# 0x002A/MuCHSALSA

Measured on AMD Instinct MI355X. Metric: overlap-pairs/s, higher is better.
Workload: dtype int32+f64; 1 GPU; 100k synthetic Nanopore x10 kb, 500k unitig anchors, 10x coverage (BASELINE.json configs[2]); rows=5059558, reads=100000, anchors=499992, edges=981460, edgematches_rank0=25532466, orders_rank0=1029308, parallelism=one job on one GPU, edges_proven_clean_rank0=5372

## Files before the change

### muchsalsa_amd/csrc/msgpu_api.hip

```cpp
#include <hip/hip_runtime.h>

#include <chrono>
#include <cmath>
#include <cstdarg>
#include <cstdio>
#include <cstdlib>
#include <cstring>
#include <condition_variable>
#include <deque>
#include <mutex>
#include <new>
#include <thread>
#include <vector>
#include <algorithm>
#include <sys/mman.h>
#include <unistd.h>

#include "asm_internal.h"
#include "host_pool.h"
#include "msgpu.h"
#include "msgpu_internal.h"
#include "msgpu_stage.h"

using namespace msgpu;
// ... 189 lines not shown
}

struct msgpu_ctx : msgpu::StageCtx {
  hipStream_t  own_stream = nullptr;
  msgpu_params p;
  State        state      = ST_CREATED;
  uint32_t     shard = 0, nshards = 1;
  uint32_t     win_lo = 0, win_hi = 0xffffffffu;
  uint64_t     base_edges = 0, base_ems = 0, base_orders = 0, base_ids = 0;
  ScalarBlock  sc;
  bool         stage_events = true;
  bool         chain_zeroed = false;
  bool         no_prologue = false;
  bool         prologue_ok = false;
  bool         scalars_clean = false;
  bool         bin_clean = false;
  size_t       bin_zero_words = 0;
  uint32_t     prologue_shard = 0, prologue_nshards = 1;
  uint64_t     prologue_own = 0;
  bool         full_scan_ok = false;
  uint64_t     index_total = 0, own_accum = 0;
  bool         nlists_clean = false;
  bool         cand_zeroed = false;
  uint64_t     prologue_bound = 0;
  uint32_t     prologue_lists[4] = {0, 0, 0, 0};
  EventHold    ev_order;
  uint32_t     decl_V = 0, decl_A = 0;
  bool                                  has_deadline = false;
  std::chrono::steady_clock::time_point deadline{};

  uint64_t n_rows = 0, n_alive = 0;
  uint32_t V = 0, A = 0;
  const msgpu_row *d_rows = nullptr;

  uint64_t n_edges = 0, n_ems = 0, n_orders = 0, n_ids = 0, n_visit = 0, total_bound = 0;
  uint32_t n_list[4] = {0, 0, 0, 0};

  DevBuf rows_in, rows_pk, cnt_read, read_off, cursor, bkt_key, bkt_dead, by_read, read_cnt, alive_rank,
      anchor_cnt, anchor_off, anchor_first, anchor_off_gen, bkt2_idx, bkt2_line, by_anchor, read_len, read_first,
      scan_tmp, vis16, spos2, visits, bin_cursor, bin_start;
  DevBuf bound, cand_off, cand_j, cand_q, scr_v2, scr_start, n_cand, n_edge, lists, edges, edge_cand;
  DevBuf big_key, big_t, big_r2s, big_pfx, pair_tab, chain_chunks, big_off, cand_sums, bucket_visits;
  EventHold ev_side[2], ev_side2;
  uint64_t    n_big_edges = 0, n_big_ems = 0;
  bool   fast_path = true;
  bool   chain_band = true;
  bool   sub_wave  = true;
  bool   use_fork  = true;
  bool   use_prologue = true;
  bool   chain_serial = false;
  uint32_t n_cls[4] = {0, 0, 0, 0};
  uint64_t n_edges_fast = 0;
  uint64_t chain_E = 0;
  DevBuf ems, order_scr, ids_scr, edge_norders, edge_nids, orders, ids, big_list, cls_list, big_elems,
      big_paths;
  DevBuf g_deg, g_off, g_adj, g_cand, g_sane, g_out;
  DevBuf sel_idx, sel_cnt, sel_off, sel_ems;

  DevBuf    alt_edges, alt_ems, alt_orders, alt_ids;
  EventHold ev_done[2], ev_copied[2];
  HostBuf   h_edges, h_ems, h_orders, h_ids, h_read_len, h_read_first, h_sel_off, h_sel_ems, h_wire[2];
  EventHold ev_part[2][3];
  std::mutex              gate_m;
  std::condition_variable gate_cv;
  uint64_t                chain_launches = 0;
  DevBuf win_cuts;
  DevBuf wire_dev[2];
  bool   wire_copy = true;

  EventHold ev[10];
  static constexpr int CK_RING = 256;
  EventHold  ck_ev[CK_RING][2];
  uint32_t   ck_head = 0, ck_count = 0;
  bool       have_index_t = false, have_cand_t = false, have_chain_t = false, index_fast = false;
  bool   have_stage_t = false;
  uint32_t index_path = 0;
  bool     index_binned = false;
  bool     use_bin = true;
  StreamHold side_stream, side_stream2, copy_stream;
  int        open() {
    own_stream = stream;
    if (int rc = sc.create()) return rc;
    const char *nf = getenv("MSGPU_NO_FASTPATH");
    fast_path      = !(nf && nf[0] == '1');
    const char *nb = getenv("MSGPU_NO_BAND");
    chain_band     = fast_path && !(nb && nb[0] == '1');
    const char *ns = getenv("MSGPU_NO_SUBWAVE");
    sub_wave       = !(ns && ns[0] == '1');
    const char *nw = getenv("MSGPU_NO_WIRE_COPY");
    wire_copy      = !(nw && nw[0] == '1');
    const char *nbin = getenv("MSGPU_NO_BIN");
    use_bin          = !(nbin && nbin[0] == '1');
    use_prologue = !getenv("MSGPU_NO_PROLOGUE");
    use_fork     = !getenv("MSGPU_NO_FORK");
    chain_serial = getenv("MSGPU_CHAIN_SERIAL") != nullptr;
    int prio_least = 0, prio_greatest = 0;
    if (hipDeviceGetStreamPriorityRange(&prio_least, &prio_greatest) != hipSuccess) prio_least = prio_greatest = 0;
    bool ok = side_stream.create(hipStreamNonBlocking, prio_greatest) == hipSuccess &&
              side_stream2.create(hipStreamNonBlocking, prio_greatest) == hipSuccess && copy_stream.create() == hipSuccess;
    for (auto &e : ev) ok = ok && e.create() == hipSuccess;
    EventHold *const untimed[] = {&ev_order, &ev_side[0], &ev_side[1], &ev_side2, &ev_done[0], &ev_done[1], &ev_copied[0], &ev_copied[1],
                                  &ev_part[0][0], &ev_part[0][1], &ev_part[0][2], &ev_part[1][0], &ev_part[1][1], &ev_part[1][2]};
    for (EventHold *e : untimed) ok = ok && e->create(hipEventDisableTiming) == hipSuccess;
    return ok ? MSGPU_OK : MSGPU_E_HIP;
  }
};

// ... 661 lines not shown
    k.pub            = publish ? c->sc.arm() : HostPublish{nullptr, 0};
    k.nlists         = scalar<unsigned long long>(c, SC_NLISTS);
    launch_emit_edges(st, k, publish);
  };
  uint64_t cap_edges = 0, cap_big = 0;
  capacities(&cap_edges, &cap_big);
  emit(cap_edges, cap_big, true);
  c->nlists_clean = true;
  STAGE_HIP(c, hipGetLastError());
  if (int rc = close_readback(c)) return rc;
  const uint64_t *tot = host_scalar<uint64_t>(c, SC_TOTAL_A), *big = host_scalar<uint64_t>(c, SC_BIGSTATS);
  c->n_big_edges = big[0];
  c->n_big_ems   = big[1];
  for (int k = 0; k < 4; ++k) c->n_cls[k] = host_scalar<uint32_t>(c, SC_CLS)[k];
  c->n_ems   = tot[0];
  c->n_edges = tot[1];
  c->n_visit = c->total_bound;
  if (c->n_edges >= 0xfffffff0ull) return fail(c, MSGPU_E_ARG, "edge table too large (%llu)", (unsigned long long)c->n_edges);
  if (c->n_edges > cap_edges || c->n_big_edges >= cap_big) {
    STAGE_HIP(c, c->edges.ensure((c->n_edges ? c->n_edges : 1) * sizeof(msgpu_edge)));
    STAGE_HIP(c, c->edge_cand.ensure((c->n_edges ? c->n_edges : 1) * 8));
    STAGE_HIP(c, c->cls_list.ensure((c->n_edges + 1) * 4));
    STAGE_HIP(c, c->big_list.ensure((c->n_big_edges + 1) * 4));
    STAGE_HIP(c, c->big_off.ensure((c->n_big_edges + 1) * 8));
    STAGE_HIP(c, c->chain_chunks.ensure(chunk_words(c->edges.room() / sizeof(msgpu_edge)) * 8));
    capacities(&cap_edges, &cap_big);
    emit(cap_edges, cap_big, false);
  }
  c->chain_zeroed = true;
  STAGE_HIP(c, hipGetLastError());
  if (c->stage_events) STAGE_HIP(c, hipEventRecord(c->ev[3], st));
  c->have_cand_t = c->stage_events;
  c->n_orders    = 0;
  c->n_ids       = 0;
  c->state       = ST_EDGES;
  return MSGPU_OK;
}

int msgpu_chaining_and_overlaps(msgpu_ctx *c) {
  if (!c) return MSGPU_E_ARG;
  if (c->state < ST_EDGES || c->state == ST_RESULT)
    return fail(c, MSGPU_E_STATE, "msgpu_chaining_and_overlaps before msgpu_calculate_edges");
  STAGE_HIP(c, hipSetDevice(c->device));
  hipStream_t    st = c->stream;
  const uint64_t E = c->n_edges, M = c->n_ems;
  for (int k = 0; k < 2; ++k)
    if (!c->ck_ev[c->ck_head][k]) STAGE_HIP(c, c->ck_ev[c->ck_head][k].create());
  const hipEvent_t ck_begin = c->ck_ev[c->ck_head][0], ck_end = c->ck_ev[c->ck_head][1];
  if (c->stage_events) STAGE_HIP(c, hipEventRecord(c->ev[4], st));

  STAGE_HIP(c, c->ems.ensure((M ? M : 1) * sizeof(msgpu_edgematch)));
  STAGE_HIP(c, c->order_scr.ensure((M ? M : 1) * sizeof(msgpu_order)));
  STAGE_HIP(c, c->ids_scr.ensure((M ? M : 1) * 4));
  STAGE_HIP(c, c->edge_norders.ensure((E + 4) * 4));
  STAGE_HIP(c, c->edge_nids.ensure((E + 4) * 4));
  STAGE_HIP(c, c->chain_chunks.ensure(chunk_words(E) * 8));

  ChainArgs a;
  a.edges        = c->edges.as<msgpu_edge>();
  a.edge_cand    = c->edge_cand.as<uint64_t>();
  a.n_edges      = E;
  a.cand_j       = c->cand_j.as<uint32_t>();
  a.cand_q       = c->cand_q.as<uint32_t>();
  a.read_off     = c->read_off.as<uint32_t>();
  a.read_cnt     = c->read_cnt.as<uint32_t>();
  a.read_len     = c->read_len.as<int32_t>();
  a.by_read      = c->by_read.as<IRow>();
  a.ems          = c->ems.as<msgpu_edgematch>();
  a.order_scr    = c->order_scr.as<msgpu_order>();
  a.ids_scr      = c->ids_scr.as<uint32_t>();
  a.edge_norders = c->edge_norders.as<uint32_t>();
  a.edge_nids    = c->edge_nids.as<uint32_t>();
  a.err          = scalar<uint32_t>(c, SC_ERR);
  if (!c->pair_tab.p) {
    STAGE_HIP(c, c->pair_tab.ensure(PAIR_TAB_WORDS * sizeof(uint32_t)));
    launch_fill_pair_tab(st, c->pair_tab.as<uint32_t>());
  }
  a.pair_tab     = c->pair_tab.as<uint32_t>();
  a.pair_tab64   = c->pair_tab.as<uint32_t>() + 4 * PAIR_TAB_STRIDE;
  a.pair_tab_sub = c->pair_tab.as<uint32_t>() + 4 * PAIR_TAB_STRIDE + 2 * PAIR_TAB_STRIDE;
  if (!c->chain_zeroed)
    STAGE_HIP(c, hipMemsetAsync(c->chain_chunks.p, 0, chunk_words(E) * 8, st));
  c->chain_zeroed = false;
  a.chunk_sums   = c->chain_chunks.as<unsigned long long>();
  a.fast_path    = (c->fast_path ? CHAIN_FAST_SHORTCUT : 0) | (c->chain_band ? CHAIN_FAST_BAND : 0);
  c->chain_E     = E;
  a.fast_margin  = static_cast<long long>(std::min<uint64_t>(c->p.wiggle_room, uint64_t(1) << 40)) - 3;
  a.wiggle       = static_cast<double>(c->p.wiggle_room);
  a.ratio_pct    = c->p.ratio_pct;
  a.alt_frac     = c->p.alt_frac;
  a.out_edge_base = static_cast<uint32_t>(c->base_edges);

  const uint32_t n_big = static_cast<uint32_t>(c->n_big_edges);
  if (n_big) {
    STAGE_HIP(c, c->big_elems.ensure((c->n_big_ems ? c->n_big_ems : 1) * big_elem_bytes()));
    STAGE_HIP(c, c->big_paths.ensure((c->n_big_ems ? c->n_big_ems : 1) * 2 * big_path_bytes()));
  }
  if (n_big) STAGE_HIP(c, hipEventRecord(c->ev_side[0], st));
  auto launch_big = [&]() -> int {
    if (!n_big) return MSGPU_OK;
    STAGE_HIP(c, hipStreamWaitEvent(c->side_stream, c->ev_side[0], 0));
    launch_chain_big(c->side_stream, a, c->big_list.as<uint32_t>(), c->big_off.as<uint64_t>(), n_big,
                     c->big_elems.p, c->big_paths.p);
    STAGE_HIP(c, hipEventRecord(c->ev_side[1], c->side_stream));
    return MSGPU_OK;
  };
  {
    std::lock_guard<std::mutex> g(c->gate_m);
    ++c->chain_launches;
  }
  c->gate_cv.notify_all();
  if (int rc = launch_big()) return rc;
  STAGE_HIP(c, hipEventRecord(ck_begin, st));
  if (c->sub_wave && E) {
    const uint32_t *list = c->cls_list.as<uint32_t>();
    const uint32_t *l64 = list, *l32 = l64 + c->n_cls[2], *l16 = l32 + c->n_cls[1], *l8 = l16 + c->n_cls[0];
    const bool serial = c->chain_serial;
    const bool any_sub = c->n_cls[0] || c->n_cls[1] || c->n_cls[3];
    const bool beside  = !serial && any_sub && c->n_cls[2];
    if (beside) STAGE_HIP(c, hipStreamWaitEvent(c->side_stream2, ck_begin, 0));
    launch_chain(st, a, l64, c->n_cls[2]);
    if (serial) {
      launch_chain_sub(st, a, 32, l32, c->n_cls[1]);
      launch_chain_sub(st, a, 16, l16, c->n_cls[0]);
      launch_chain_sub(st, a, 8, l8, c->n_cls[3]);
    } else if (any_sub) {
      launch_chain_sub_all(beside ? c->side_stream2 : st, a, l32, c->n_cls[1], l16, c->n_cls[0], l8, c->n_cls[3]);
    }
    if (beside) {
      STAGE_HIP(c, hipEventRecord(c->ev_side2, c->side_stream2));
      STAGE_HIP(c, hipStreamWaitEvent(st, c->ev_side2, 0));
    }
  } else {
    launch_chain(st, a, nullptr, 0);
  }
  STAGE_HIP(c, hipEventRecord(ck_end, st));
  c->ck_head = (c->ck_head + 1) % msgpu_ctx::CK_RING;
  if (c->ck_count < msgpu_ctx::CK_RING) ++c->ck_count;
  STAGE_HIP(c, hipGetLastError());
  if (n_big) STAGE_HIP(c, hipStreamWaitEvent(st, c->ev_side[1], 0));

  if (c->stage_events) STAGE_HIP(c, hipEventRecord(c->ev[7], st));
  auto compact = [&](bool publish) {
    CompactArgs k;
    k.edges        = c->edges.as<msgpu_edge>();
    k.n_edges      = E;
    k.edge_norders = c->edge_norders.as<uint32_t>();
    k.edge_nids    = c->edge_nids.as<uint32_t>();
    k.chunk_sums   = c->chain_chunks.as<unsigned long long>();
    k.n_chunks     = static_cast<uint32_t>((E + COMPACT_CHUNK - 1) / COMPACT_CHUNK);
    k.scalars      = c->sc.d;
    k.pub          = publish ? c->sc.arm() : HostPublish{nullptr, 0};
    k.order_scr    = c->order_scr.as<msgpu_order>();
    k.ids_scr      = c->ids_scr.as<uint32_t>();
    k.orders       = c->orders.as<msgpu_order>();
    k.ids          = c->ids.as<uint32_t>();
    k.out_em_base    = c->base_ems;
    k.out_order_base = c->base_orders;
    k.out_ids_base   = c->base_ids;
    k.out_edge_base  = static_cast<uint32_t>(c->base_edges);
    k.cap_orders     = c->orders.room() / sizeof(msgpu_order);
    k.cap_ids        = c->ids.room() / 4;
    launch_compact(st, k);
  };
  const uint64_t cap_orders = c->orders.room() / sizeof(msgpu_order), cap_ids = c->ids.room() / 4;
  compact(true);
  STAGE_HIP(c, hipGetLastError());
  if (int rc = close_readback(c)) return rc;
  c->n_edges_fast     = *host_scalar<uint64_t>(c, SC_TOTAL_C);
  const uint64_t *tot = host_scalar<uint64_t>(c, SC_TOTAL_A);
  c->n_orders = tot[0];
  c->n_ids    = tot[1];
  if (c->n_orders > cap_orders || c->n_ids > cap_ids) {
    STAGE_HIP(c, c->orders.ensure((c->n_orders ? c->n_orders : 1) * sizeof(msgpu_order)));
    STAGE_HIP(c, c->ids.ensure((c->n_ids ? c->n_ids : 1) * 4));
    compact(false);
  }
  STAGE_HIP(c, hipGetLastError());
  if (c->stage_events) STAGE_HIP(c, hipEventRecord(c->ev[8], st));
  c->have_chain_t = true;
  c->have_stage_t = c->stage_events;
  c->state        = ST_CHAINED;
  return MSGPU_OK;
}

int msgpu_set_stage_events(msgpu_ctx *c, int on) {
  if (!c) return MSGPU_E_ARG;
  c->stage_events = on != 0;
  return MSGPU_OK;
}

int msgpu_get_counts(msgpu_ctx *c, msgpu_counts *out) {
  if (!c || !out) return MSGPU_E_ARG;
  memset(out, 0, sizeof(*out));
  out->n_rows_in       = c->n_rows;
  out->n_rows_alive    = c->n_alive;
  out->n_reads         = c->V;
  out->n_anchors       = c->A;
  out->n_edges         = c->state >= ST_EDGES ? c->n_edges : 0;
  out->n_ems           = c->state >= ST_EDGES ? c->n_ems : 0;
  out->n_orders        = c->state >= ST_CHAINED ? c->n_orders : 0;
// ... 757 lines not shown
```

### muchsalsa_amd/csrc/msgpu_internal.h

```cpp
#ifndef MSGPU_INTERNAL_H
#define MSGPU_INTERNAL_H

#include <hip/hip_runtime.h>
#include <stdint.h>

#include "msgpu.h"

namespace msgpu {

struct IRow {
  int32_t  n_lo, n_hi, i_lo, i_hi;
  uint32_t score, line, other, pf;
};
static_assert(sizeof(IRow) == 32, "IRow must be 32 bytes");
struct SRow {
  int32_t  i_lo, i_hi;
  uint32_t read, pf;
};
static_assert(sizeof(SRow) == 16, "SRow must be 16 bytes");
constexpr uint32_t PF_POS_MASK = 0x3fffffffu;
constexpr uint32_t PF_DIR      = 1u << 30;
constexpr uint32_t PF_PRIM     = 1u << 31;

enum { SC_MAXIDS = 0 , SC_ERR = 1, SC_TOTAL_A = 2, SC_TOTAL_B = 3, SC_TOTAL_C = 4, SC_NLISTS = 5 ,
// ... 17 lines not shown
  const uint32_t *read_off, *read_cnt, *anchor_off;
  const IRow     *by_read;
  const SRow     *by_anchor;
  const uint4    *vis;
  const uint64_t *cand_off;
  uint32_t       *cand_j;
  uint32_t       *cand_q;
  uint32_t       *edge_scr_v2;
  uint32_t       *edge_scr_start;
  uint32_t       *n_cand, *n_edge;
  unsigned long long *big_stats;
  uint32_t        th_overlap;
};
constexpr uint32_t CAND_CHUNK = 256;
struct CandZero {
  uint32_t *n_cand, *n_edge;
  uint32_t *scalar_words;
  uint32_t  n_scalar_words;
};
struct EmitArgs {
  const uint32_t *n_edge, *n_cand;
  const uint64_t *cand_off;
  const uint32_t *edge_scr_v2, *edge_scr_start;
  uint32_t        V;
  const uint32_t *hist;
  const unsigned long long *chunk_sums;
  uint32_t        n_chunks;
  msgpu_edge     *edges;
  uint64_t       *edge_cand;
  uint32_t       *list;
  uint32_t       *big_list;
  uint64_t       *big_off;
  unsigned long long *big_cursor;
  const unsigned long long *big_stats;
  uint64_t        cap_edges, cap_big;
  unsigned long long *chain_chunk_sums;
  uint32_t        n_chain_chunk_words;
  uint64_t       *scalars;
  HostPublish     pub;
  unsigned long long *nlists;
};

struct ChainArgs {
  msgpu_edge      *edges;
  const uint64_t  *edge_cand;
  uint64_t         n_edges;
  const uint32_t  *cand_j, *cand_q;
  const uint32_t  *read_off, *read_cnt;
  const int32_t   *read_len;
  const IRow      *by_read;
  msgpu_edgematch *ems;
  msgpu_order     *order_scr;
  uint32_t        *ids_scr;
  uint32_t        *edge_norders, *edge_nids;
  uint32_t        *err;
  const uint32_t  *pair_tab;
  const uint32_t  *pair_tab64;
  const uint32_t  *pair_tab_sub;
  unsigned long long *chunk_sums;
  int              fast_path;
  long long        fast_margin;
  double           wiggle, ratio_pct, alt_frac;
  uint32_t         out_edge_base;
};

constexpr uint32_t COMPACT_CHUNK = 1024;
struct CompactArgs {
  msgpu_edge        *edges;
  uint64_t           n_edges;
  const uint32_t    *edge_norders, *edge_nids;
  const unsigned long long *chunk_sums;
  uint32_t           n_chunks;
  uint64_t          *scalars;
  HostPublish        pub;
  const msgpu_order *order_scr;
  const uint32_t    *ids_scr;
  msgpu_order       *orders;
  uint32_t          *ids;
  uint64_t           out_em_base, out_order_base, out_ids_base;
  uint32_t           out_edge_base;
  uint64_t           cap_orders, cap_ids;
};

constexpr uint32_t MAX_WORLD = 64;
struct MergeBase {
  uint64_t edges, orders, ids;
  uint32_t read_id, anchor_id;
};
struct MergeArgs {
  const uint8_t *gathered;
  uint64_t       slab_bytes, off_edges, off_orders, off_ids;
  uint32_t       world;
  MergeBase      base[MAX_WORLD + 1];
  msgpu_edge    *edges;
  msgpu_order   *orders;
  uint32_t      *ids;
};

struct PackWireArgs {
  const msgpu_edge  *edges;
  const msgpu_order *orders;
  const uint32_t    *ids;
  uint64_t           n_edges, n_orders, n_ids;
  uint8_t           *w_edges, *w_orders;
  uint32_t          *w_ids;
  uint64_t           base_ems = 0, base_orders = 0, base_ids = 0;
  uint32_t           base_edges = 0;
};
inline uint64_t wire_edges_bytes(uint64_t n) { return 17 * n + 8; }
inline uint64_t wire_orders_bytes(uint64_t n) { return 33 * n + 4; }
inline uint64_t wire_ids_bytes(uint64_t n, uint32_t id_bytes) { return id_bytes == 3 ? (3 * n + 3) / 4 * 4 : 4 * n; }
struct WindowCutArgs {
  uint32_t n;
  float    frac[255];
};
void launch_window_cuts(hipStream_t st, const uint64_t *cum, uint32_t V, const WindowCutArgs &a, uint64_t *out);
void launch_pack_wire(hipStream_t st, const PackWireArgs &a);
void unpack_wire_host(const uint8_t *w_edges, const uint8_t *w_orders, const uint32_t *w_ids, uint32_t id_bytes, uint64_t n_edges,
                      uint64_t n_orders, uint64_t n_ids, uint64_t base_edges, uint64_t base_ems, uint64_t base_orders,
                      uint64_t base_ids, msgpu_edge *edges, msgpu_order *orders, uint32_t *ids, unsigned threads, unsigned tables = 7);
void launch_merge_wire(hipStream_t st, const MergeArgs &a, bool ids3);

template <class T> void exclusive_scan(hipStream_t st, const uint32_t *in, uint64_t n, T *out, T *block_sums, T *d_total);
// ... 148 lines not shown
```

### muchsalsa_amd/csrc/msgpu_kernels.hip

```cpp
#include <hip/hip_runtime.h>
#include <stdint.h>
#include <stdlib.h>

#include <type_traits>
#include <utility>

#include "msgpu.h"
#include "msgpu_internal.h"
#include "msgpu_device.h"

namespace msgpu {


constexpr int SCAN_ITEMS = 8;
uint32_t      scan_blocks(uint64_t n);

template <class T> __global__ __launch_bounds__(256) void k_scan_reduce(const uint32_t *in, uint64_t n, T *block_sums) {
  __shared__ T s[4];
  uint64_t     base = static_cast<uint64_t>(blockIdx.x) * 256 * SCAN_ITEMS;
  T            sum  = 0;
  for (int i = 0; i < SCAN_ITEMS; ++i) {
    uint64_t idx = base + static_cast<uint64_t>(i) * 256 + threadIdx.x;
    if (idx < n) sum += in[idx];
  }
// ... 1246 lines not shown
    const uint32_t e = sub;
    st_r[round] = en_r[round] = v2_r[round] = 0;
    if (e < ne_r4[round]) {
      st_r[round] = a.edge_scr_start[co_r[round] + e];
      en_r[round] = (e + 1 < ne_r4[round]) ? a.edge_scr_start[co_r[round] + e + 1] : nc_r4[round];
      v2_r[round] = a.edge_scr_v2[co_r[round] + e];
    }
  }
#pragma unroll
  for (int round = 0; round < ROUNDS; ++round) {
    const uint32_t lr = round * 64 + (threadIdx.x >> 4), r = chunk * CAND_CHUNK + lr;
    const uint32_t ne = ne_r4[round];
    if (ne == 0) continue;
    const uint32_t nc = nc_r4[round];
    const uint64_t eb = base_e + s_eb[lr], mb = base_m + s_mb[lr], co = co_r[round];
    for (uint32_t e = sub; e < ne; e += 16) {
      const bool     first = e == static_cast<uint32_t>(sub);
      const uint32_t st = first ? st_r[round] : a.edge_scr_start[co + e];
      const uint32_t en = first ? en_r[round] : ((e + 1 < ne) ? a.edge_scr_start[co + e + 1] : nc);
      msgpu_edge     ed;
      ed.v1        = r;
      ed.v2        = first ? v2_r[round] : a.edge_scr_v2[co + e];
      ed.em_off    = mb + st;
      ed.order_off = 0;
      ed.em_cnt    = en - st;
      ed.order_cnt = 0;
      ed.shadow    = 0;
      ed.pad       = 0;
      a.edges[eb + e]     = ed;
      a.edge_cand[eb + e] = co + st;
      if (ed.em_cnt > 64) {
        const unsigned long long i = atomicAdd(&a.big_cursor[0], 1ull);
        a.big_list[i] = static_cast<uint32_t>(eb + e);
        a.big_off[i]  = atomicAdd(&a.big_cursor[1], static_cast<unsigned long long>(ed.em_cnt));
      } else if (ed.em_cnt) {
        a.list[atomicAdd(&s_pos[ed.em_cnt - 1], 1u)] = static_cast<uint32_t>(eb + e);
      }
    }
  }
}
void launch_emit_edges(hipStream_t st, const EmitArgs &a, bool reduce) {
  if (reduce && a.n_chunks)
    hipLaunchKernelGGL(k_cand_reduce, dim3(a.n_chunks), dim3(1024), 0, st, a.n_edge, a.n_cand, a.cand_off, a.edge_scr_start, a.V,
                       const_cast<unsigned long long *>(a.chunk_sums), const_cast<uint32_t *>(a.hist));
  hipLaunchKernelGGL(k_emit_edges, dim3(a.n_chunks ? a.n_chunks : 1), dim3(1024), 0, st, a);
}


__device__ __forceinline__ void chunk_add(unsigned long long *chunk_sums, uint64_t e, bool clean, uint32_t n_orders, uint32_t n_ids, bool banded = false) {
  static_assert(COMPACT_CHUNK < (1u << 16), "two 16-bit edge counts in the low half of a chunk sum");
  unsigned long long *c = chunk_sums + 2 * (e / COMPACT_CHUNK);
  __hip_atomic_fetch_add(c, (clean ? 1ull : 0ull) | (banded ? 1ull << 16 : 0ull) | (static_cast<unsigned long long>(n_orders) << 32), __ATOMIC_RELAXED, __HIP_MEMORY_SCOPE_AGENT);
  __hip_atomic_fetch_add(c + 1, static_cast<unsigned long long>(n_ids), __ATOMIC_RELAXED, __HIP_MEMORY_SCOPE_AGENT);
}
__device__ __forceinline__ void band_fallback_add(unsigned long long *chunk_sums, uint64_t n_edges) {
  __hip_atomic_fetch_add(chunk_sums + 2 * (n_edges / COMPACT_CHUNK + 1), 1ull, __ATOMIC_RELAXED, __HIP_MEMORY_SCOPE_AGENT);
}

struct PathRec {
  uint64_t mask;
  uint64_t score;
  uint32_t primary;
  uint32_t pad;
};

struct __attribute__((aligned(16))) ChainElem {
  double clo1, chi1;
  double clo2, chi2;
  int    rlo1, rhi1, rlo2, rhi2;
};

struct NanoMasks {
  unsigned long long pos, neg, ovl, abort_;
};
template <bool WF, int SORTED >
__device__ __forceinline__ NanoMasks nano_check(double k_clo, double k_chi, double l_clo, double l_chi, int k_rlo,
                                                int k_rhi, int l_rlo, int l_rhi, double &d) {
  typedef unsigned long long M;
  const bool lt_lo_b = k_clo < l_clo;
  const M    lt_lo = __ballot(lt_lo_b), lt_hi = __ballot(k_chi < l_chi);
  const M    gt_lo = __ballot(k_clo > l_clo), gt_hi = __ballot(k_chi > l_chi);
  NanoMasks  f;
  const double x = k_chi - l_clo;
  const double y = l_chi - k_clo;
  double       t = lt_lo_b ? x : y;
  if (WF) {
    f.ovl = __ballot(t >= 0.0);
    d     = fabs(t) + 1;
  } else {
    f.ovl = __ballot(k_clo <= l_chi) & __ballot(l_clo <= k_chi);
    t     = __builtin_amdgcn_inverse_ballot_w64(f.ovl) ? t : -t;
    d = t + 1;
  }
  if (WF) {
    f.pos = lt_lo & lt_hi;
    f.neg = gt_lo & gt_hi;
  } else {
    f.pos = lt_lo & (lt_hi | ~f.ovl);
    f.neg = (f.ovl & gt_lo & gt_hi) | ~(f.ovl | lt_lo);
  }
  if (SORTED == 1) {
    const M rovl = __ballot(l_rlo <= k_rhi);
    const M u2   = __ballot(k_rlo < l_rlo) & __ballot(k_rhi < l_rhi);
    f.abort_     = rovl & (f.neg | (f.pos & ~u2));
  } else if (SORTED == 2) {
    const M rovl = __ballot(k_rlo <= l_rhi);
// ... 433 lines not shown
        R2 = rl_f64(clo2, l);
      }
      bool     have = false;
      uint32_t fl   = 0;
      double   lo = 0, ro = 0;
      if (L1 <= L2 && R1 <= R2) {
        have = true;
        fl   = MSGPU_ORD_START_V1 | MSGPU_ORD_CONTAINED;
        lo   = L2 - L1;
        ro   = R2 - R1;
      } else if (L1 >= L2 && R1 >= R2) {
        have = true;
        fl   = MSGPU_ORD_CONTAINED;
        lo   = L1 - L2;
        ro   = R1 - R2;
      } else if (L1 > L2 && R1 < R2) {
        have = true;
        fl   = MSGPU_ORD_START_V1;
        lo   = L1 - L2;
        ro   = R2 - R1;
      } else if (L1 < L2 && R1 > R2) {
        have = true;
        fl   = 0;
        lo   = L2 - L1;
        ro   = R1 - R2;
      }
      if (!have) continue;
      const uint32_t cnt = static_cast<uint32_t>(__popcll(mask));
      if ((mask >> lane) & 1ull) {
        const uint32_t pos = static_cast<uint32_t>(__popcll(mask & ((1ull << lane) - 1)));
        a.ids_scr[ed.em_off + n_ids + pos] = anchor;
      }
      if (lane == 0) {
        msgpu_order o;
        o.edge_idx     = static_cast<uint32_t>(e);
        o.flags        = fl | (dir ? MSGPU_ORD_DIR : 0u) | (pv[pi].primary ? MSGPU_ORD_PRIMARY : 0u);
        o.left_offset  = lo;
        o.right_offset = ro;
        o.score        = pv[pi].score;
        o.ids_off      = n_ids;
        o.ids_cnt      = cnt;
        o.start        = (fl & MSGPU_ORD_START_V1) ? v1 : v2;
        o.end          = (fl & MSGPU_ORD_START_V1) ? v2 : v1;
        o.base         = v1;
        o.pad[0]       = 0;
        o.pad[1]       = 0;
        a.order_scr[ed.em_off + n_orders] = o;
      }
      ++n_orders;
      n_ids += cnt;
    }
  }
  if (lane == 0) {
    a.edge_norders[e] = n_orders;
    a.edge_nids[e]    = n_ids;
    a.edges[e].shadow = shadow ? 1 : 0;
    chunk_add(a.chunk_sums, e, clean, n_orders, n_ids, banded);
  }
}


struct __attribute__((aligned(16))) SubPath {
  uint32_t mask, primary;
  uint64_t score;
};

__device__ __forceinline__ double shfl_f64(double v, int src) {
  const long long b  = __double_as_longlong(v);
  const uint32_t  lo = __shfl(static_cast<uint32_t>(b), src), hi = __shfl(static_cast<uint32_t>(b >> 32), src);
  return __longlong_as_double(static_cast<long long>((static_cast<unsigned long long>(hi) << 32) | lo));
}

template <int W> __device__ __forceinline__ uint32_t group_bits(unsigned long long m, int gbase) {
  return static_cast<uint32_t>(m >> gbase) & (W == 32 ? 0xffffffffu : ((1u << W) - 1u));
}

template <int W> __device__ __forceinline__ int longest_prefix(unsigned long long m) {
#pragma unroll
  for (int d = 32; d >= W; d >>= 1) m |= m >> d;
  return __popc(static_cast<uint32_t>(m) & (W == 32 ? 0xffffffffu : ((1u << W) - 1u)));
}

template <int K> __device__ __forceinline__ uint32_t row_bcast(uint32_t v) {
  static_assert(K >= 0 && K < 16, "row lane");
  return static_cast<uint32_t>(__builtin_amdgcn_mov_dpp(static_cast<int>(v), 0x150 + K, 0xf, 0xf, false));
}

template <int W, int K> __device__ __forceinline__ uint32_t group_bcast(uint32_t v) {
  static_assert(K >= 0 && K < W, "group lane");
  if constexpr (W == 16) {
    return row_bcast<K>(v);
  } else if constexpr (W == 8) {
    const int lo = __builtin_amdgcn_mov_dpp(static_cast<int>(v), 0x150 + K, 0xf, 0x3, false);
    return static_cast<uint32_t>(__builtin_amdgcn_update_dpp(lo, static_cast<int>(v), 0x150 + 8 + K, 0xf, 0xc, false));
  } else if constexpr (K < 16) {
    const int r = static_cast<int>(row_bcast<K>(v));
    return static_cast<uint32_t>(__builtin_amdgcn_update_dpp(r, r, 0x142, 0xa, 0xf, false));
  } else {
    const uint32_t r  = row_bcast<K - 16>(v);
    const uint32_t ro = static_cast<uint32_t>(__builtin_amdgcn_mov_dpp(static_cast<int>(v), 0x150 + K - 16, 0xa, 0xf, false));
    return __builtin_amdgcn_permlane16_swap(r, ro, false, false)[1];
  }
}
template <int W, int K> __device__ __forceinline__ double group_bcast_f64(double v) {
  const unsigned long long b  = __builtin_bit_cast(unsigned long long, v);
  const uint32_t           lo = group_bcast<W, K>(static_cast<uint32_t>(b));
  const uint32_t           hi = group_bcast<W, K>(static_cast<uint32_t>(b >> 32));
  return __builtin_bit_cast(double, (static_cast<unsigned long long>(hi) << 32) | lo);
}
// ... 387 lines not shown
      const double  *kf = s_keep[wave][gbase + f], *kl = s_keep[wave][gbase + l];
      const double   L1 = kf[0], R1 = kl[2];
      const double   L2 = dir ? kf[1] : kf[3], R2 = dir ? kl[3] : kl[1];
      bool     have = false;
      uint32_t fl   = 0;
      double   lo = 0, ro = 0;
      if (L1 <= L2 && R1 <= R2) {
        have = true;
        fl   = MSGPU_ORD_START_V1 | MSGPU_ORD_CONTAINED;
        lo   = L2 - L1;
        ro   = R2 - R1;
      } else if (L1 >= L2 && R1 >= R2) {
        have = true;
        fl   = MSGPU_ORD_CONTAINED;
        lo   = L1 - L2;
        ro   = R1 - R2;
      } else if (L1 > L2 && R1 < R2) {
        have = true;
        fl   = MSGPU_ORD_START_V1;
        lo   = L1 - L2;
        ro   = R2 - R1;
      } else if (L1 < L2 && R1 > R2) {
        have = true;
        fl   = 0;
        lo   = L2 - L1;
        ro   = R1 - R2;
      }
      const bool emit = has && have;
      if (emit) {
        const uint32_t cnt = static_cast<uint32_t>(__popc(mask));
        if ((mask >> sl) & 1u) a.ids_scr[ed.em_off + n_ids + static_cast<uint32_t>(__popc(mask & ((1u << sl) - 1u)))] = s_anchor[wave][lane];
        if (sl == 0) {
          msgpu_order o;
          o.edge_idx     = e;
          o.flags        = fl | (dir ? MSGPU_ORD_DIR : 0u) | (rec.primary ? MSGPU_ORD_PRIMARY : 0u);
          o.left_offset  = lo;
          o.right_offset = ro;
          o.score        = rec.score;
          o.ids_off      = n_ids;
          o.ids_cnt      = cnt;
          o.start        = (fl & MSGPU_ORD_START_V1) ? v1 : v2;
          o.end          = (fl & MSGPU_ORD_START_V1) ? v2 : v1;
          o.base         = v1;
          o.pad[0]       = 0;
          o.pad[1]       = 0;
          a.order_scr[ed.em_off + n_orders] = o;
        }
        ++n_orders;
        n_ids += cnt;
      }
    }
  }
  if (n && sl == 0) {
    a.edge_norders[e] = n_orders;
    a.edge_nids[e]    = n_ids;
    a.edges[e].shadow = shadow ? 1 : 0;
    chunk_add(a.chunk_sums, e, clean, n_orders, n_ids);
  }
}

template <int W>
__global__ __launch_bounds__(256) __attribute__((amdgpu_waves_per_eu(W == 32 ? 7 : 6, W == 32 ? 7 : 6))) void k_chain_sub(ChainArgs a, const uint32_t *list, uint32_t n_list) {
  __shared__ __attribute__((aligned(16))) unsigned char s_wavebuf[4][sizeof(ChainElem) * 64];
  __shared__ uint32_t                                  s_cm[4][64];
  __shared__ __attribute__((aligned(16))) double       s_keep[4][64][4];
  __shared__ uint32_t                                  s_anchor[4][64];
  chain_sub_body<W>(a, list, n_list, blockIdx.x, s_wavebuf, s_cm, s_keep, s_anchor);
}
#ifndef MSGPU_SUB_WAVES
#define MSGPU_SUB_WAVES 7
#endif
__global__ __launch_bounds__(256) __attribute__((amdgpu_waves_per_eu(MSGPU_SUB_WAVES, MSGPU_SUB_WAVES))) void k_chain_sub_all(ChainArgs a, ChainSubLists l) {
  __shared__ __attribute__((aligned(16))) unsigned char s_wavebuf[4][sizeof(ChainElem) * 64];
  __shared__ uint32_t                                  s_cm[4][64];
  __shared__ __attribute__((aligned(16))) double       s_keep[4][64][4];
  __shared__ uint32_t                                  s_anchor[4][64];
  uint32_t b = blockIdx.x;
  if (b < l.nb32) {
    chain_sub_body<32>(a, l.list32, l.n32, b, s_wavebuf, s_cm, s_keep, s_anchor);
  } else if ((b -= l.nb32) < l.nb16) {
    chain_sub_body<16>(a, l.list16, l.n16, b, s_wavebuf, s_cm, s_keep, s_anchor);
  } else {
    chain_sub_body<8>(a, l.list8, l.n8, b - l.nb16, s_wavebuf, s_cm, s_keep, s_anchor);
  }
}
template __global__ void k_chain_sub<8>(ChainArgs, const uint32_t *, uint32_t);
template __global__ void k_chain_sub<16>(ChainArgs, const uint32_t *, uint32_t);
template __global__ void k_chain_sub<32>(ChainArgs, const uint32_t *, uint32_t);


struct BigElem {
  int      rlo1, rhi1, rlo2, rhi2;
  double   clo1, chi1, clo2, chi2, ovr1, ovr2, score;
  uint32_t anchor, j1, q2, flags;
  double   pop;
  uint32_t pred, used;
};

struct BigPath {
  uint32_t end, first, len, primary;
  uint64_t score;
};

struct BigHot {
  int    rlo1, rhi1, rlo2, rhi2;
  double clo1, chi1, clo2, chi2;
};
template <class EK, class EL>
__device__ __forceinline__ bool big_compat(const EK &K, const EL &L, bool direction, double wiggle, double ratio_pct) {
// ... 361 lines not shown
        const uint32_t f = pv[pi].first, l = pv[pi].end;
        const double   L1 = E[f].clo1, R1 = E[l].ovr1;
        double         L2 = E[f].clo2, R2 = E[l].ovr2;
        if (!dir) {
          L2 = E[f].ovr2;
          R2 = E[l].clo2;
        }
        bool     have = false;
        uint32_t fl   = 0;
        double   lo = 0, ro = 0;
        if (L1 <= L2 && R1 <= R2) {
          have = true;
          fl   = MSGPU_ORD_START_V1 | MSGPU_ORD_CONTAINED;
          lo   = L2 - L1;
          ro   = R2 - R1;
        } else if (L1 >= L2 && R1 >= R2) {
          have = true;
          fl   = MSGPU_ORD_CONTAINED;
          lo   = L1 - L2;
          ro   = R1 - R2;
        } else if (L1 > L2 && R1 < R2) {
          have = true;
          fl   = MSGPU_ORD_START_V1;
          lo   = L1 - L2;
          ro   = R2 - R1;
        } else if (L1 < L2 && R1 > R2) {
          have = true;
          fl   = 0;
          lo   = L2 - L1;
          ro   = R1 - R2;
        }
        if (!have) continue;
        const uint32_t cnt = pv[pi].len;
        uint32_t       w   = cnt;
        for (uint32_t c = l; c != 0xffffffffu; c = PRED(c)) a.ids_scr[ed.em_off + n_ids + --w] = E[c].anchor;
        msgpu_order o;
        o.edge_idx     = static_cast<uint32_t>(e);
        o.flags        = fl | (dir ? MSGPU_ORD_DIR : 0u) | (pv[pi].primary ? MSGPU_ORD_PRIMARY : 0u);
        o.left_offset  = lo;
        o.right_offset = ro;
        o.score        = pv[pi].score;
        o.ids_off      = n_ids;
        o.ids_cnt      = cnt;
        o.start        = (fl & MSGPU_ORD_START_V1) ? v1 : v2;
        o.end          = (fl & MSGPU_ORD_START_V1) ? v2 : v1;
        o.base         = v1;
        o.pad[0]       = 0;
        o.pad[1]       = 0;
        a.order_scr[ed.em_off + n_orders] = o;
        ++n_orders;
        n_ids += cnt;
      }
    }
    a.edge_norders[e] = n_orders;
    a.edge_nids[e]    = n_ids;
    a.edges[e].shadow = shadow ? 1 : 0;
    chunk_add(a.chunk_sums, e, false, n_orders, n_ids);
  }
}

__device__ __forceinline__ void tab64_entry(uint32_t *tab, int p, int k, int l, int run) {
  (void)run;
  tab[4 * PAIR_TAB_STRIDE + 2 * p]     = static_cast<uint32_t>(k * 48);
  tab[4 * PAIR_TAB_STRIDE + 2 * p + 1] = static_cast<uint32_t>(l * 48);
}
__device__ __forceinline__ void tabsub_entry(uint32_t *tab, int t, int p, int k, int l, int run) {
  uint32_t *e = tab + 4 * PAIR_TAB_STRIDE + 2 * PAIR_TAB_STRIDE + (static_cast<size_t>(t - 1) * PAIR_TAB_STRIDE + p) * 2;
  e[0]        = static_cast<uint32_t>(k * 48) | (static_cast<uint32_t>(l * 48) << 16);
  e[1]        = static_cast<uint32_t>(k) | (static_cast<uint32_t>(run) << 8) | (static_cast<uint32_t>(l * 4) << 16);
}
__device__ __forceinline__ void band64_entry(uint32_t *tab, int p) {
  constexpr int B = MSGPU_CHAIN_BAND, TRI = B * (B + 1) / 2;
  int k = 0, l = 1;
  if (p < TRI) {
    l = static_cast<int>((1.0f + __fsqrt_rn(1.0f + 8.0f * static_cast<float>(p))) * 0.5f);
    if (l * (l - 1) / 2 > p) --l;
    if ((l + 1) * l / 2 <= p) ++l;
    k = p - l * (l - 1) / 2;
  } else {
    const int q = p - TRI;
    l = B + 1 + q / B;
    k = l - B + q % B;
    if (l >= 64) {
      k = 0;
      l = 1;
    }
  }
  tab[PAIR_TAB_BAND64_OFF + 2 * p]     = static_cast<uint32_t>(k * 48);
  tab[PAIR_TAB_BAND64_OFF + 2 * p + 1] = static_cast<uint32_t>(l * 48);
}
__global__ __launch_bounds__(256) void k_fill_pair_tab(uint32_t *tab) {
  const int i = blockIdx.x * 256 + threadIdx.x;
  if (i >= 4 * static_cast<int>(PAIR_TAB_STRIDE)) return;
  const int t = i / static_cast<int>(PAIR_TAB_STRIDE), p = i % static_cast<int>(PAIR_TAB_STRIDE), W = 64 >> t;
  if (t == 0) band64_entry(tab, p);
  if (p >= 2016) {
    tab[i] = 1u << 8;
    if (t == 0) tab64_entry(tab, p, 0, 1, 0);
    else tabsub_entry(tab, t, p, 0, 1, 0);
    return;
  }
  int l = static_cast<int>((1.0f + __fsqrt_rn(1.0f + 8.0f * static_cast<float>(p))) * 0.5f);
  if (l * (l - 1) / 2 > p) --l;
  if ((l + 1) * l / 2 <= p) ++l;
  const int k = p - l * (l - 1) / 2, lane = p % W;
  const int run = (k == 0 || lane == 0) ? min(l - k, W - lane) : 0;
  tab[i] = static_cast<uint32_t>(k | (l << 8) | (run << 16)) | (static_cast<uint32_t>(64 - run - k) << 24);
  if (t == 0) tab64_entry(tab, p, k, l, run);
  else tabsub_entry(tab, t, p, k, l, run);
}

__global__ __launch_bounds__(1024) __attribute__((amdgpu_waves_per_eu(8, 8))) void k_compact(CompactArgs a) {
  __shared__ unsigned long long s_red[16][5], s_tot[5], s_em[COMPACT_CHUNK];
  __shared__ uint32_t           s_ob[COMPACT_CHUNK], s_ib[COMPACT_CHUNK], s_no[COMPACT_CHUNK], s_w[2][16];
  static_assert(COMPACT_CHUNK == 1024, "an edge per thread");
  const int      lane = threadIdx.x & 63, wave = threadIdx.x >> 6;
  const uint32_t chunk = blockIdx.x;
  const uint64_t my_e  = static_cast<uint64_t>(chunk) * COMPACT_CHUNK + threadIdx.x;
  const uint32_t my_no = my_e < a.n_edges ? a.edge_norders[my_e] : 0u, my_ni = my_e < a.n_edges ? a.edge_nids[my_e] : 0u;
  const uint64_t my_em = my_e < a.n_edges ? a.edges[my_e].em_off : 0ull;
  unsigned long long t[5] = {0, 0, 0, 0, 0};
  for (uint32_t c = threadIdx.x; c < a.n_chunks; c += 1024) {
    const unsigned long long w0 = a.chunk_sums[2 * c], w1 = a.chunk_sums[2 * c + 1];
    const unsigned long long no = w0 >> 32, nf = w0 & 0xffffull;
    if (c < chunk) {
      t[0] += no;
      t[1] += w1;
    }
    t[2] += no;
    t[3] += w1;
    t[4] += nf;
  }
#pragma unroll
  for (int k = 0; k < 5; ++k) {
    for (int d = 32; d > 0; d >>= 1) t[k] += __shfl_xor(t[k], d);
    if (lane == 0) s_red[wave][k] = t[k];
  }
  __syncthreads();
  if (wave == 0) {
#pragma unroll
    for (int k = 0; k < 5; ++k) {
      unsigned long long v = lane < 16 ? s_red[lane][k] : 0ull;
      for (int d = 8; d > 0; d >>= 1) v += __shfl_xor(v, d);
      if (lane == 0) s_tot[k] = v;
    }
  }
  __syncthreads();
  const unsigned long long base_o = s_tot[0], base_i = s_tot[1], tot_o = s_tot[2], tot_i = s_tot[3], tot_f = s_tot[4];
  if (chunk == 0 && a.scalars && threadIdx.x < 64) {
    if (lane == 0) {
      a.scalars[SC_TOTAL_A] = tot_o;
      a.scalars[SC_TOTAL_B] = tot_i;
      a.scalars[SC_TOTAL_C] = tot_f;
    }
    publish_to_host(a.pub, lane, lane == SC_TOTAL_A ? tot_o : lane == SC_TOTAL_B ? tot_i : lane == SC_TOTAL_C ? tot_f : lane < SC_COUNT ? a.scalars[lane] : 0ull);
  }
  if (tot_o > a.cap_orders || tot_i > a.cap_ids) return;
  const uint64_t e0 = static_cast<uint64_t>(chunk) * COMPACT_CHUNK;
  if (e0 >= a.n_edges) return;
  {
    const uint32_t no = my_no, ni = my_ni;
    const uint64_t em = my_em;
    const uint32_t io = wave_incl_scan(no), ii = wave_incl_scan(ni);
    if (lane == 63) {
      s_w[0][wave] = io;
      s_w[1][wave] = ii;
    }
    __syncthreads();
    uint32_t bo = io - no, bi = ii - ni;
    for (int w = 0; w < wave; ++w) {
      bo += s_w[0][w];
      bi += s_w[1][w];
    }
    s_ob[threadIdx.x] = bo;
    s_ib[threadIdx.x] = bi;
    s_no[threadIdx.x] = no;
    s_em[threadIdx.x] = em;
  }
  __syncthreads();
  constexpr int ROUNDS = COMPACT_CHUNK / 256;
  const int     sub = lane & 3;
#pragma unroll 1
  for (int round = 0; round < ROUNDS; ++round) {
    const uint32_t le   = round * 256 + wave * 16 + (lane >> 2);
    const uint64_t e    = e0 + le;
    const bool     have = e < a.n_edges;
    const uint32_t no   = have ? s_no[le] : 0u;
    const uint64_t em_off = s_em[le];
    uint64_t       oo = 0, io = 0;
    if (have) {
      oo = base_o + s_ob[le];
      io = base_i + s_ib[le];
      if (sub == 0) {
        a.edges[e].order_off = oo + a.out_order_base;
        a.edges[e].order_cnt = static_cast<uint16_t>(no);
        a.edges[e].em_off    = em_off + a.out_em_base;
      }
    }
    uint32_t max_no = no;
    for (int d = 32; d >= 4; d >>= 1) max_no = max(max_no, static_cast<uint32_t>(__shfl_xor(static_cast<int>(max_no), d)));
    for (uint32_t i = 0; i < max_no; ++i) {
      const bool on = i < no;
      uint4      w  = make_uint4(0, 0, 0, 0);
      if (on) w = reinterpret_cast<const uint4 *>(&a.order_scr[em_off + i])[sub];
      const int      q2  = (lane & ~3) + 2;
      const uint32_t rel = static_cast<uint32_t>(__shfl(static_cast<int>(w.x), q2));
      const uint32_t cnt = static_cast<uint32_t>(__shfl(static_cast<int>(w.z), q2));
      if (sub == 2) {
        const uint64_t gio = io + a.out_ids_base;
        w.x = static_cast<uint32_t>(gio);
        w.y = static_cast<uint32_t>(gio >> 32);
      }
      if (sub == 0) w.x += a.out_edge_base;
      if (on) {
        reinterpret_cast<uint4 *>(&a.orders[oo + i])[sub] = w;
        for (uint32_t q = sub; q < cnt; q += 4) a.ids[io + q] = a.ids_scr[em_off + rel + q];
        io += cnt;
      }
    }
  }
}


__global__ __launch_bounds__(256) void k_merge_gathered(MergeArgs a) {
  const uint64_t i = static_cast<uint64_t>(blockIdx.x) * 256 + threadIdx.x;
  const uint64_t nE = a.base[a.world].edges, nO = a.base[a.world].orders, nI = a.base[a.world].ids;
  if (i < nE) {
    uint32_t r = 0;
    while (i >= a.base[r + 1].edges) ++r;
    const uint64_t    k  = i - a.base[r].edges;
    const msgpu_edge *src = reinterpret_cast<const msgpu_edge *>(a.gathered + r * a.slab_bytes + a.off_edges);
    msgpu_edge        e  = src[k];
    e.order_off += a.base[r].orders;
    e.v1 += a.base[r].read_id;
    e.v2 += a.base[r].read_id;
    a.edges[i] = e;
  }
  if (i < nO) {
    uint32_t r = 0;
    while (i >= a.base[r + 1].orders) ++r;
    const uint64_t     k   = i - a.base[r].orders;
    const msgpu_order *src = reinterpret_cast<const msgpu_order *>(a.gathered + r * a.slab_bytes + a.off_orders);
    msgpu_order        o   = src[k];
    o.edge_idx += static_cast<uint32_t>(a.base[r].edges);
    o.ids_off += a.base[r].ids;
    o.start += a.base[r].read_id;
    o.end += a.base[r].read_id;
    o.base += a.base[r].read_id;
    a.orders[i] = o;
  }
  if (i < nI) {
    uint32_t r = 0;
    while (i >= a.base[r + 1].ids) ++r;
    const uint64_t  k   = i - a.base[r].ids;
    const uint32_t *src = reinterpret_cast<const uint32_t *>(a.gathered + r * a.slab_bytes + a.off_ids);
    a.ids[i]            = src[k] + a.base[r].anchor_id;
  }
}


struct WireEdges {
  const uint32_t *em_off, *order_off, *v1, *v2;
  const uint8_t  *shadow;
  __device__ WireEdges(const uint8_t *p, uint64_t n) {
    em_off    = reinterpret_cast<const uint32_t *>(p);
    order_off = em_off + (n + 1);
    v1        = order_off + (n + 1);
    v2        = v1 + n;
    shadow    = reinterpret_cast<const uint8_t *>(v2 + n);
  }
};
// ... 308 lines not shown
```

Measured before the change: 458.9 million overlap-pairs/s.

## Pack per-edge counts into edge record and flatten compact copy via binary search

Chain kernels now write order/id counts and the shadow flag directly into the second 16-byte half of each edge record, removing the separate edge_norders/edge_nids arrays and their allocations. k_compact reads each edge as two uint4 loads, then replaces the per-edge serial loop (bounded by the max order count in a quad) with a flat, load-balanced copy. Each thread binary-searches the prefix sums in shared memory to find its source edge for every order and id element, with unrolled batches. This removes load imbalance and divergent per-edge loops in exchange for log-depth LDS searches per element and a changed meaning for edge fields during the intermediate stage.

```diff
diff --git a/muchsalsa_amd/csrc/msgpu_api.hip b/muchsalsa_amd/csrc/msgpu_api.hip
--- a/muchsalsa_amd/csrc/msgpu_api.hip
+++ b/muchsalsa_amd/csrc/msgpu_api.hip
@@ -265,7 +265,7 @@
   uint32_t n_cls[4] = {0, 0, 0, 0};
   uint64_t n_edges_fast = 0;
   uint64_t chain_E = 0;
-  DevBuf ems, order_scr, ids_scr, edge_norders, edge_nids, orders, ids, big_list, cls_list, big_elems,
+  DevBuf ems, order_scr, ids_scr, orders, ids, big_list, cls_list, big_elems,
       big_paths;
   DevBuf g_deg, g_off, g_adj, g_cand, g_sane, g_out;
   DevBuf sel_idx, sel_cnt, sel_off, sel_ems;
@@ -1033,8 +1033,6 @@
   STAGE_HIP(c, c->ems.ensure((M ? M : 1) * sizeof(msgpu_edgematch)));
   STAGE_HIP(c, c->order_scr.ensure((M ? M : 1) * sizeof(msgpu_order)));
   STAGE_HIP(c, c->ids_scr.ensure((M ? M : 1) * 4));
-  STAGE_HIP(c, c->edge_norders.ensure((E + 4) * 4));
-  STAGE_HIP(c, c->edge_nids.ensure((E + 4) * 4));
   STAGE_HIP(c, c->chain_chunks.ensure(chunk_words(E) * 8));
 
   ChainArgs a;
@@ -1050,8 +1048,6 @@
   a.ems          = c->ems.as<msgpu_edgematch>();
   a.order_scr    = c->order_scr.as<msgpu_order>();
   a.ids_scr      = c->ids_scr.as<uint32_t>();
-  a.edge_norders = c->edge_norders.as<uint32_t>();
-  a.edge_nids    = c->edge_nids.as<uint32_t>();
   a.err          = scalar<uint32_t>(c, SC_ERR);
   if (!c->pair_tab.p) {
     STAGE_HIP(c, c->pair_tab.ensure(PAIR_TAB_WORDS * sizeof(uint32_t)));
@@ -1126,8 +1122,6 @@
     CompactArgs k;
     k.edges        = c->edges.as<msgpu_edge>();
     k.n_edges      = E;
-    k.edge_norders = c->edge_norders.as<uint32_t>();
-    k.edge_nids    = c->edge_nids.as<uint32_t>();
     k.chunk_sums   = c->chain_chunks.as<unsigned long long>();
     k.n_chunks     = static_cast<uint32_t>((E + COMPACT_CHUNK - 1) / COMPACT_CHUNK);
     k.scalars      = c->sc.d;
diff --git a/muchsalsa_amd/csrc/msgpu_internal.h b/muchsalsa_amd/csrc/msgpu_internal.h
--- a/muchsalsa_amd/csrc/msgpu_internal.h
+++ b/muchsalsa_amd/csrc/msgpu_internal.h
@@ -93,7 +93,6 @@
   msgpu_edgematch *ems;
   msgpu_order     *order_scr;
   uint32_t        *ids_scr;
-  uint32_t        *edge_norders, *edge_nids;
   uint32_t        *err;
   const uint32_t  *pair_tab;
   const uint32_t  *pair_tab64;
@@ -109,7 +108,6 @@
 struct CompactArgs {
   msgpu_edge        *edges;
   uint64_t           n_edges;
-  const uint32_t    *edge_norders, *edge_nids;
   const unsigned long long *chunk_sums;
   uint32_t           n_chunks;
   uint64_t          *scalars;
diff --git a/muchsalsa_amd/csrc/msgpu_kernels.hip b/muchsalsa_amd/csrc/msgpu_kernels.hip
--- a/muchsalsa_amd/csrc/msgpu_kernels.hip
+++ b/muchsalsa_amd/csrc/msgpu_kernels.hip
@@ -1322,6 +1322,9 @@
   unsigned long long *c = chunk_sums + 2 * (e / COMPACT_CHUNK);
   __hip_atomic_fetch_add(c, (clean ? 1ull : 0ull) | (banded ? 1ull << 16 : 0ull) | (static_cast<unsigned long long>(n_orders) << 32), __ATOMIC_RELAXED, __HIP_MEMORY_SCOPE_AGENT);
   __hip_atomic_fetch_add(c + 1, static_cast<unsigned long long>(n_ids), __ATOMIC_RELAXED, __HIP_MEMORY_SCOPE_AGENT);
+}
+__device__ __forceinline__ void edge_counts(msgpu_edge *edges, uint64_t e, uint32_t em_cnt, uint32_t n_orders, uint32_t n_ids, bool shadow) {
+  reinterpret_cast<uint4 *>(&edges[e])[1] = make_uint4(n_ids, 0u, em_cnt, (n_orders & 0xffffu) | (shadow ? 1u << 16 : 0u));
 }
 __device__ __forceinline__ void band_fallback_add(unsigned long long *chunk_sums, uint64_t n_edges) {
   __hip_atomic_fetch_add(chunk_sums + 2 * (n_edges / COMPACT_CHUNK + 1), 1ull, __ATOMIC_RELAXED, __HIP_MEMORY_SCOPE_AGENT);
@@ -1861,9 +1864,7 @@
     }
   }
   if (lane == 0) {
-    a.edge_norders[e] = n_orders;
-    a.edge_nids[e]    = n_ids;
-    a.edges[e].shadow = shadow ? 1 : 0;
+    edge_counts(a.edges, e, n, n_orders, n_ids, shadow);
     chunk_add(a.chunk_sums, e, clean, n_orders, n_ids, banded);
   }
 }
@@ -2357,9 +2358,7 @@
     }
   }
   if (n && sl == 0) {
-    a.edge_norders[e] = n_orders;
-    a.edge_nids[e]    = n_ids;
-    a.edges[e].shadow = shadow ? 1 : 0;
+    edge_counts(a.edges, e, n, n_orders, n_ids, shadow);
     chunk_add(a.chunk_sums, e, clean, n_orders, n_ids);
   }
 }
@@ -2827,9 +2826,7 @@
         n_ids += cnt;
       }
     }
-    a.edge_norders[e] = n_orders;
-    a.edge_nids[e]    = n_ids;
-    a.edges[e].shadow = shadow ? 1 : 0;
+    edge_counts(a.edges, e, n, n_orders, n_ids, shadow);
     chunk_add(a.chunk_sums, e, false, n_orders, n_ids);
   }
 }
@@ -2885,15 +2882,30 @@
   else tabsub_entry(tab, t, p, k, l, run);
 }
 
+
+__device__ __forceinline__ uint32_t compact_find(const uint32_t *tab, uint32_t x) {
+  uint32_t le = 0;
+#pragma unroll
+  for (uint32_t s = COMPACT_CHUNK / 2; s; s >>= 1)
+    if (tab[le + s] <= x) le += s;
+  return le;
+}
 __global__ __launch_bounds__(1024) __attribute__((amdgpu_waves_per_eu(8, 8))) void k_compact(CompactArgs a) {
   __shared__ unsigned long long s_red[16][5], s_tot[5], s_em[COMPACT_CHUNK];
-  __shared__ uint32_t           s_ob[COMPACT_CHUNK], s_ib[COMPACT_CHUNK], s_no[COMPACT_CHUNK], s_w[2][16];
+  __shared__ uint32_t           s_ob[COMPACT_CHUNK + 1], s_ib[COMPACT_CHUNK + 1], s_w[2][16];
   static_assert(COMPACT_CHUNK == 1024, "an edge per thread");
   const int      lane = threadIdx.x & 63, wave = threadIdx.x >> 6;
   const uint32_t chunk = blockIdx.x;
-  const uint64_t my_e  = static_cast<uint64_t>(chunk) * COMPACT_CHUNK + threadIdx.x;
-  const uint32_t my_no = my_e < a.n_edges ? a.edge_norders[my_e] : 0u, my_ni = my_e < a.n_edges ? a.edge_nids[my_e] : 0u;
-  const uint64_t my_em = my_e < a.n_edges ? a.edges[my_e].em_off : 0ull;
+  const uint64_t my_e = static_cast<uint64_t>(chunk) * COMPACT_CHUNK + threadIdx.x;
+  uint4          my_lo = make_uint4(0, 0, 0, 0), my_hi = make_uint4(0, 0, 0, 0);
+  if (my_e < a.n_edges) {
+    const uint4 *p = reinterpret_cast<const uint4 *>(&a.edges[my_e]);
+    my_lo          = p[0];
+    my_hi          = p[1];
+  }
+  static_assert(sizeof(msgpu_edge) == 32 && offsetof(msgpu_edge, em_off) == 8 && offsetof(msgpu_edge, order_off) == 16 &&
+                    offsetof(msgpu_edge, em_cnt) == 24 && offsetof(msgpu_edge, order_cnt) == 28,
+                "the edge record as two 16-byte halves");
   unsigned long long t[5] = {0, 0, 0, 0, 0};
   for (uint32_t c = threadIdx.x; c < a.n_chunks; c += 1024) {
     const unsigned long long w0 = a.chunk_sums[2 * c], w1 = a.chunk_sums[2 * c + 1];
@@ -2934,8 +2946,8 @@
   const uint64_t e0 = static_cast<uint64_t>(chunk) * COMPACT_CHUNK;
   if (e0 >= a.n_edges) return;
   {
-    const uint32_t no = my_no, ni = my_ni;
-    const uint64_t em = my_em;
+    const uint32_t no = my_hi.w & 0xffffu, ni = my_hi.x;
+    const uint64_t em = static_cast<uint64_t>(my_lo.z) | (static_cast<uint64_t>(my_lo.w) << 32);
     const uint32_t io = wave_incl_scan(no), ii = wave_incl_scan(ni);
     if (lane == 63) {
       s_w[0][wave] = io;
@@ -2949,49 +2961,65 @@
     }
     s_ob[threadIdx.x] = bo;
     s_ib[threadIdx.x] = bi;
-    s_no[threadIdx.x] = no;
     s_em[threadIdx.x] = em;
+    if (threadIdx.x == COMPACT_CHUNK - 1) {
+      s_ob[COMPACT_CHUNK] = bo + no;
+      s_ib[COMPACT_CHUNK] = bi + ni;
+    }
+    if (my_e < a.n_edges) {
+      const uint64_t oo = base_o + bo + a.out_order_base;
+      reinterpret_cast<uint4 *>(&a.edges[my_e])[1] = make_uint4(static_cast<uint32_t>(oo), static_cast<uint32_t>(oo >> 32), my_hi.z, my_hi.w);
+      if (a.out_em_base) a.edges[my_e].em_off = em + a.out_em_base;
+    }
   }
   __syncthreads();
-  constexpr int ROUNDS = COMPACT_CHUNK / 256;
-  const int     sub = lane & 3;
-#pragma unroll 1
-  for (int round = 0; round < ROUNDS; ++round) {
-    const uint32_t le   = round * 256 + wave * 16 + (lane >> 2);
-    const uint64_t e    = e0 + le;
-    const bool     have = e < a.n_edges;
-    const uint32_t no   = have ? s_no[le] : 0u;
-    const uint64_t em_off = s_em[le];
-    uint64_t       oo = 0, io = 0;
-    if (have) {
-      oo = base_o + s_ob[le];
-      io = base_i + s_ib[le];
-      if (sub == 0) {
-        a.edges[e].order_off = oo + a.out_order_base;
-        a.edges[e].order_cnt = static_cast<uint16_t>(no);
-        a.edges[e].em_off    = em_off + a.out_em_base;
-      }
-    }
-    uint32_t max_no = no;
-    for (int d = 32; d >= 4; d >>= 1) max_no = max(max_no, static_cast<uint32_t>(__shfl_xor(static_cast<int>(max_no), d)));
-    for (uint32_t i = 0; i < max_no; ++i) {
-      const bool on = i < no;
-      uint4      w  = make_uint4(0, 0, 0, 0);
-      if (on) w = reinterpret_cast<const uint4 *>(&a.order_scr[em_off + i])[sub];
-      const int      q2  = (lane & ~3) + 2;
-      const uint32_t rel = static_cast<uint32_t>(__shfl(static_cast<int>(w.x), q2));
-      const uint32_t cnt = static_cast<uint32_t>(__shfl(static_cast<int>(w.z), q2));
-      if (sub == 2) {
-        const uint64_t gio = io + a.out_ids_base;
-        w.x = static_cast<uint32_t>(gio);
-        w.y = static_cast<uint32_t>(gio >> 32);
-      }
-      if (sub == 0) w.x += a.out_edge_base;
-      if (on) {
-        reinterpret_cast<uint4 *>(&a.orders[oo + i])[sub] = w;
-        for (uint32_t q = sub; q < cnt; q += 4) a.ids[io + q] = a.ids_scr[em_off + rel + q];
-        io += cnt;
-      }
+  const uint32_t n_o = s_ob[COMPACT_CHUNK], n_i = s_ib[COMPACT_CHUNK];
+  constexpr uint32_t ORD_U = 4, IDS_U = 8;
+  if (n_o) {
+    const uint32_t sub = threadIdx.x & 3, sl = threadIdx.x >> 2;
+    for (uint32_t s0 = 0;;) {
+      const uint32_t rem = n_o - s0;
+      uint4          w[ORD_U];
+      uint32_t       ib[ORD_U];
+#pragma unroll
+      for (uint32_t k = 0; k < ORD_U; ++k) {
+        const uint32_t s  = s0 + min(k * (COMPACT_CHUNK / 4) + sl, rem - 1);
+        const uint32_t le = compact_find(s_ob, s);
+        w[k]  = reinterpret_cast<const uint4 *>(&a.order_scr[s_em[le] + (s - s_ob[le])])[sub];
+        ib[k] = s_ib[le];
+      }
+#pragma unroll
+      for (uint32_t k = 0; k < ORD_U; ++k) {
+        const uint32_t off = k * (COMPACT_CHUNK / 4) + sl;
+        if (sub == 0) w[k].x += a.out_edge_base;
+        if (sub == 2) {
+          const uint64_t gio = a.out_ids_base + base_i + ib[k] + w[k].x;
+          w[k].x = static_cast<uint32_t>(gio);
+          w[k].y = static_cast<uint32_t>(gio >> 32);
+        }
+        if (off < rem) reinterpret_cast<uint4 *>(&a.orders[base_o + s0 + off])[sub] = w[k];
+      }
+      if (rem <= ORD_U * (COMPACT_CHUNK / 4)) break;
+      s0 += ORD_U * (COMPACT_CHUNK / 4);
+    }
+  }
+  if (n_i) {
+    for (uint32_t q0 = 0;;) {
+      const uint32_t rem = n_i - q0;
+      uint32_t       v[IDS_U];
+#pragma unroll
+      for (uint32_t k = 0; k < IDS_U; ++k) {
+        const uint32_t q  = q0 + min(k * COMPACT_CHUNK + threadIdx.x, rem - 1);
+        const uint32_t le = compact_find(s_ib, q);
+        v[k] = a.ids_scr[s_em[le] + (q - s_ib[le])];
+      }
+#pragma unroll
+      for (uint32_t k = 0; k < IDS_U; ++k) {
+        const uint32_t off = k * COMPACT_CHUNK + threadIdx.x;
+        if (off < rem) a.ids[base_i + q0 + off] = v[k];
+      }
+      if (rem <= IDS_U * COMPACT_CHUNK) break;
+      q0 += IDS_U * COMPACT_CHUNK;
     }
   }
 }
```

Measured after the change: 471.2 million overlap-pairs/s, median of 6. 1.03x the previous value.
